# samiwilf/torchrec-oldfork

Hardware: AMD Instinct MI355X
Metric: samples/sec Criteo-1TB DLRM batch 65536 (higher is better)
Workload: dtype f32; 1 GPU; DLRM Criteo-1TB shape: 26 tables (177.9M rows, 84.85 GiB fp32, D=128), 13 dense, pooling factor 1, dense 512-256-128, over 1024-1024-512-256-1, fused exact SGD; global_batch=65536, local_batch=65536, parallelism=mp1: 26 table-wise + 0 row-wise + 0 replicated (data-parallel) tables, dense dp1, ids=uniform, distinct_batches=32, seed=0, data_ranks=1

## Files before the change

include/tbe_hip.h:

```cpp
#ifndef TBE_HIP_H_
#define TBE_HIP_H_

#include <stddef.h>
#include <stdint.h>

#ifdef __cplusplus
extern "C" {
#endif

#define TBE_OK 0
#define TBE_ERR_INVALID_ARGUMENT (-1)
#define TBE_ERR_LAUNCH (-2)
#define TBE_ERR_WORKSPACE (-3)
#define TBE_ERR_UNSUPPORTED (-4)

#define TBE_POOL_SUM 0
#define TBE_POOL_MEAN 1
#define TBE_POOL_NONE 2

#define TBE_OPT_EXACT_SGD 0
#define TBE_OPT_EXACT_ROWWISE_ADAGRAD 1
#define TBE_OPT_ADAM 2
#define TBE_OPT_EXACT_ADAGRAD 3
#define TBE_OPT_DENSE_GRAD 100
// ... 145 lines not shown

int tbe_dlrm_interaction_forward_f32(const float* dense, const float* sparse, int32_t B,
                                     int32_t F, int32_t D, float* out, int64_t out_row_stride,
                                     void* stream);
int tbe_dlrm_interaction_backward_f32(const float* dense, const float* sparse,
                                      const float* grad_out, int64_t grad_row_stride, int32_t B, int32_t F, int32_t D,
                                      float* grad_dense, float* grad_sparse, void* stream);

size_t tbe_relu_backward_bias_grad_workspace_bytes(int64_t B, int32_t N);
int tbe_relu_backward_bias_grad_f32(const float* grad_out, const float* act, int64_t B, int32_t N,
                                    float* grad_in, float* bias_grad, void* workspace,
                                    size_t workspace_bytes, void* stream);

size_t tbe_weighted_colsum_workspace_bytes(int64_t B, int32_t N);
int tbe_weighted_colsum_f32(const float* x, const float* w, int64_t B, int32_t N, float* out,
                            void* workspace, size_t workspace_bytes, void* stream);

int64_t tbe_colsum_row_blocks(int64_t B, int32_t N);
int tbe_relu_backward_bias_partials_f32(const float* grad_out, const float* act, int64_t B, int32_t N,
                                        float* grad_in, float* partial, size_t partial_bytes, void* stream);
int tbe_weighted_colsum_partials_f32(const float* x, const float* w, int64_t B, int32_t N, float* partial,
                                     size_t partial_bytes, void* stream);

int tbe_multi_chunk_sum_f32(const int64_t* seg_table, int32_t nseg, int64_t max_numel, float* dst, float scale,
                            void* stream);
int tbe_multi_chunk_sum_host_table_f32(const int64_t* host_seg_table, int32_t nseg, int64_t max_numel, float* dst,
                                       float scale, void* stream);

size_t tbe_bce_with_logits_workspace_bytes(void);
int tbe_bce_with_logits_f32(const float* logits, const void* labels, int32_t label_elem_size, int64_t B, float* loss,
                            float* dlogits, void* workspace, size_t workspace_bytes, void* stream);

int tbe_jagged_2d_to_dense_f32(const float* values, const int64_t* offsets, int32_t B,
                               int32_t D, int32_t max_L, float* dense, void* stream);

int tbe_dense_to_jagged_2d_f32(const float* dense, const int64_t* offsets, int32_t B, int32_t D,
                               int32_t max_L, int64_t N, float* values, void* stream);

int tbe_offsets_range(const int64_t* offsets, int64_t n, int64_t range_size, int64_t* out,
                      void* stream);

int tbe_copy_rows(const void* src, int64_t src_rows, const int32_t* rows, int32_t n_rows,
                  int64_t row_bytes, void* dst, void* stream);

#ifdef __cplusplus
}
// ... 3 lines not shown
```

torchrec-oldfork_amd/csrc/mlp_epilogue.hip:

```cpp
#include <algorithm>
#include <cstring>

#include "common.hpp"

namespace tbe {

__host__ __device__ inline int rows_per_block(int N) { return N >= 512 ? 256 : 64; }

template <int TX>
__global__ __launch_bounds__(256) void drelu_bgrad_kernel(const float* __restrict__ gy, const float* __restrict__ act,
                                                          float* __restrict__ gx, float* __restrict__ partial,
                                                          int64_t B, int N) {
  constexpr int TY = 256 / TX;
  __shared__ float4 red[TY][TX];
  const int tx = threadIdx.x % TX;
  const int ty = threadIdx.x / TX;
  const int col = (blockIdx.x * TX + tx) * 4;
  const int rpb = rows_per_block(N);
  const int64_t row0 = static_cast<int64_t>(blockIdx.y) * rpb;
  const int64_t row1 = min(B, row0 + rpb);
  float4 acc = make_float4(0.f, 0.f, 0.f, 0.f);
  if (col < N) {
#pragma unroll 4
    for (int64_t r = row0 + ty; r < row1; r += TY) {
// ... 219 lines not shown
    }
  }
  red[threadIdx.x] = acc;
  __syncthreads();
  for (int o = 128; o > 0; o >>= 1) {
    if (static_cast<int>(threadIdx.x) < o) red[threadIdx.x] += red[threadIdx.x + o];
    __syncthreads();
  }
  if (threadIdx.x == 0) {
    __hip_atomic_store(&partial[blockIdx.x], red[0], __ATOMIC_RELAXED, __HIP_MEMORY_SCOPE_AGENT);
    __threadfence();
    is_last = atomicAdd(ticket, 1u) == static_cast<unsigned>(nblk - 1);
  }
  __syncthreads();
  if (is_last && threadIdx.x == 0) {
    __threadfence();
    float tot = 0.f;
    for (int b = 0; b < nblk; ++b) tot += __hip_atomic_load(&partial[b], __ATOMIC_RELAXED, __HIP_MEMORY_SCOPE_AGENT);
    *loss = tot * invB;
    *ticket = 0u;
  }
}

}

using namespace tbe;

extern "C" size_t tbe_relu_backward_bias_grad_workspace_bytes(int64_t B, int32_t N) {
  if (B <= 0 || N <= 0) return 256;
  const int rpb = rows_per_block(N);
  return align_up(static_cast<size_t>((B + rpb - 1) / rpb) * N * sizeof(float), 256);
}

extern "C" int tbe_relu_backward_bias_grad_f32(const float* grad_out, const float* act, int64_t B, int32_t N,
                                               float* grad_in, float* bias_grad, void* workspace,
                                               size_t workspace_bytes, void* stream) {
  TBE_REQUIRE(B >= 0 && N > 0 && (N & 3) == 0, "tbe_relu_backward_bias_grad_f32: N=%d must be a positive multiple of 4", N);
  TBE_REQUIRE(bias_grad != nullptr, "tbe_relu_backward_bias_grad_f32: null bias_grad");
  hipStream_t st = static_cast<hipStream_t>(stream);
  if (B == 0) {
    if (hipMemsetAsync(bias_grad, 0, sizeof(float) * N, st) != hipSuccess) return TBE_ERR_LAUNCH;
    return TBE_OK;
  }
  TBE_REQUIRE(grad_out && act && grad_in && workspace, "tbe_relu_backward_bias_grad_f32: null pointer");
  TBE_REQUIRE(((reinterpret_cast<uintptr_t>(grad_out) | reinterpret_cast<uintptr_t>(act) |
                reinterpret_cast<uintptr_t>(grad_in) | reinterpret_cast<uintptr_t>(workspace)) & 15) == 0,
// ... 88 lines not shown

extern "C" int tbe_weighted_colsum_partials_f32(const float* x, const float* w, int64_t B, int32_t N, float* partial,
                                                size_t partial_bytes, void* stream) {
  TBE_REQUIRE(B > 0 && N > 0 && (N & 3) == 0, "tbe_weighted_colsum_partials_f32: B > 0 and N a positive multiple of 4 required");
  TBE_REQUIRE(x && w && partial, "tbe_weighted_colsum_partials_f32: null pointer");
  TBE_REQUIRE(((reinterpret_cast<uintptr_t>(x) | reinterpret_cast<uintptr_t>(partial)) & 15) == 0,
              "tbe_weighted_colsum_partials_f32: tensors must be 16-B aligned");
  const int64_t nrb = tbe_colsum_row_blocks(B, N);
  TBE_REQUIRE(nrb <= 65535, "tbe_weighted_colsum_partials_f32: B=%lld too large", (long long)B);
  TBE_REQUIRE(partial_bytes >= static_cast<size_t>(nrb) * N * sizeof(float), "tbe_weighted_colsum_partials_f32: partial too small");
  hipStream_t st = static_cast<hipStream_t>(stream);
  const int vecs = N / 4;
  if (vecs >= 64) {
    hipLaunchKernelGGL(wcolsum_kernel<64>, dim3((vecs + 63) / 64, static_cast<unsigned>(nrb)), dim3(256), 0, st, x, w, partial, B, N);
  } else if (vecs >= 32) {
    hipLaunchKernelGGL(wcolsum_kernel<32>, dim3((vecs + 31) / 32, static_cast<unsigned>(nrb)), dim3(256), 0, st, x, w, partial, B, N);
  } else {
    hipLaunchKernelGGL(wcolsum_kernel<16>, dim3((vecs + 15) / 16, static_cast<unsigned>(nrb)), dim3(256), 0, st, x, w, partial, B, N);
  }
  TBE_CHECK_LAUNCH("tbe_weighted_colsum_partials_f32");
  return TBE_OK;
}

extern "C" int tbe_multi_chunk_sum_f32(const int64_t* seg_table, int32_t nseg, int64_t max_numel, float* dst, float scale,
                                       void* stream) {
  TBE_REQUIRE(nseg >= 0 && max_numel >= 0, "tbe_multi_chunk_sum_f32: bad sizes");
  if (nseg == 0 || max_numel == 0) return TBE_OK;
  TBE_REQUIRE(seg_table && dst, "tbe_multi_chunk_sum_f32: null pointer");
  TBE_REQUIRE(nseg <= 65535, "tbe_multi_chunk_sum_f32: more than 65535 segments");
  static_assert(sizeof(ChunkSeg) == 4 * sizeof(int64_t), "segment table layout");
  const int64_t tiles = (max_numel + 255) / 256;
  TBE_REQUIRE(tiles < (1ll << 31), "tbe_multi_chunk_sum_f32: segment too long");
  hipLaunchKernelGGL(multi_chunk_sum_kernel, dim3(static_cast<unsigned>(tiles), static_cast<unsigned>(nseg)), dim3(256), 0,
                     static_cast<hipStream_t>(stream), reinterpret_cast<const ChunkSeg*>(seg_table), dst, scale);
  TBE_CHECK_LAUNCH("tbe_multi_chunk_sum_f32");
  return TBE_OK;
}

extern "C" int tbe_multi_chunk_sum_host_table_f32(const int64_t* host_seg_table, int32_t nseg, int64_t max_numel, float* dst,
                                                  float scale, void* stream) {
  TBE_REQUIRE(nseg >= 0 && nseg <= kChunkSegsByValue && max_numel >= 0,
              "tbe_multi_chunk_sum_host_table_f32: 0 <= nseg <= %d required", kChunkSegsByValue);
  if (nseg == 0 || max_numel == 0) return TBE_OK;
  TBE_REQUIRE(host_seg_table != nullptr, "tbe_multi_chunk_sum_host_table_f32: null table");
  ChunkSegs32 segs{};
  memcpy(segs.s, host_seg_table, static_cast<size_t>(nseg) * sizeof(ChunkSeg));
// ... 31 lines not shown
```

torchrec-oldfork_amd/fbgemm_gpu/_lib.py:

```python
import ctypes
import os
from typing import Optional

import torch

_HERE = os.path.dirname(os.path.abspath(__file__))
LIB_PATH = os.path.normpath(os.path.join(_HERE, "..", "lib", "libtbe_hip.so"))

c_void_p = ctypes.c_void_p
c_i32 = ctypes.c_int32
c_i64 = ctypes.c_int64
c_size = ctypes.c_size_t
c_float = ctypes.c_float


class OptimizerArgs(ctypes.Structure):

    _fields_ = [
        ("optimizer", c_i32),
        ("learning_rate", c_float),
        ("eps", c_float),
        ("weight_decay", c_float),
        ("beta1", c_float),
        ("beta2", c_float),
# ... 88 lines not shown
    "tbe_pooled_exchange_unpack": (
        ctypes.c_int,
        [c_void_p, c_void_p, c_void_p, c_void_p, c_void_p, c_void_p, c_void_p, c_i32, c_i32, c_i32,
         c_i32, c_i32, c_float, c_void_p]),
    "tbe_pooled_exchange_pack": (
        ctypes.c_int,
        [c_void_p, c_void_p, c_void_p, c_void_p, c_void_p, c_void_p, c_void_p, c_i32, c_i32, c_i32,
         c_i32, c_i32, c_float, c_void_p]),
    "tbe_dlrm_interaction_forward_f32": (
        ctypes.c_int, [c_void_p, c_void_p, c_i32, c_i32, c_i32, c_void_p, c_i64, c_void_p]),
    "tbe_dlrm_interaction_backward_f32": (
        ctypes.c_int, [c_void_p, c_void_p, c_void_p, c_i64, c_i32, c_i32, c_i32, c_void_p, c_void_p, c_void_p]),
    "tbe_relu_backward_bias_grad_workspace_bytes": (c_size, [c_i64, c_i32]),
    "tbe_relu_backward_bias_grad_f32": (
        ctypes.c_int, [c_void_p, c_void_p, c_i64, c_i32, c_void_p, c_void_p, c_void_p, c_size, c_void_p]),
    "tbe_weighted_colsum_workspace_bytes": (c_size, [c_i64, c_i32]),
    "tbe_weighted_colsum_f32": (
        ctypes.c_int, [c_void_p, c_void_p, c_i64, c_i32, c_void_p, c_void_p, c_size, c_void_p]),
    "tbe_colsum_row_blocks": (c_i64, [c_i64, c_i32]),
    "tbe_relu_backward_bias_partials_f32": (
        ctypes.c_int, [c_void_p, c_void_p, c_i64, c_i32, c_void_p, c_void_p, c_size, c_void_p]),
    "tbe_weighted_colsum_partials_f32": (
        ctypes.c_int, [c_void_p, c_void_p, c_i64, c_i32, c_void_p, c_size, c_void_p]),
    "tbe_multi_chunk_sum_f32": (ctypes.c_int, [c_void_p, c_i32, c_i64, c_void_p, c_float, c_void_p]),
    "tbe_multi_chunk_sum_host_table_f32": (ctypes.c_int, [c_void_p, c_i32, c_i64, c_void_p, c_float, c_void_p]),
    "tbe_bce_with_logits_workspace_bytes": (c_size, []),
    "tbe_bce_with_logits_f32": (
        ctypes.c_int, [c_void_p, c_void_p, c_i32, c_i64, c_void_p, c_void_p, c_void_p, c_size, c_void_p]),
    "tbe_jagged_2d_to_dense_f32": (
        ctypes.c_int, [c_void_p, c_void_p, c_i32, c_i32, c_i32, c_void_p, c_void_p]),
    "tbe_dense_to_jagged_2d_f32": (
        ctypes.c_int, [c_void_p, c_void_p, c_i32, c_i32, c_i32, c_i64, c_void_p, c_void_p]),
    "tbe_offsets_range": (ctypes.c_int, [c_void_p, c_i64, c_i64, c_void_p, c_void_p]),
    "tbe_copy_rows": (ctypes.c_int, [c_void_p, c_i64, c_void_p, c_i32, c_i64, c_void_p, c_void_p]),
}

_lib: Optional[ctypes.CDLL] = None


def load() -> ctypes.CDLL:
    global _lib
    if _lib is not None:
        return _lib
    if not os.path.exists(LIB_PATH):
        raise ImportError(
            f"{LIB_PATH} is missing: the MI355X HIP extension has not been built. "
# ... 76 lines not shown
```

torchrec-oldfork_amd/torchrec_amd/distributed/_device_ops.py:

```python
import torch

from fbgemm_gpu import _lib
from fbgemm_gpu._lib import check, ptr, require_gpu, stream_ptr

_def = torch.library.Library("tbe_hip", "DEF")
_def.define("pooled_exchange_unpack(Tensor recv, Tensor feat_out_col, Tensor feat_src, Tensor feat_slab_col, "
            "Tensor slab_offset, Tensor slab_stride, int B_local, int D_total, bool vec, float scale) -> Tensor")
_def.define("pooled_exchange_unpack_into(Tensor recv, Tensor feat_out_col, Tensor feat_src, Tensor feat_slab_col, "
            "Tensor slab_offset, Tensor slab_stride, int B_local, int D_total, bool vec, float scale, Tensor(a!) out) -> Tensor(a!)")
_def.define("pooled_exchange_pack(Tensor grad, Tensor feat_out_col, Tensor feat_src, Tensor feat_slab_col, "
            "Tensor slab_offset, Tensor slab_stride, int numel, bool vec, float scale) -> Tensor")
_def.define("pooled_exchange_pack_into(Tensor grad, Tensor feat_out_col, Tensor feat_src, Tensor feat_slab_col, "
            "Tensor slab_offset, Tensor slab_stride, bool vec, float scale, Tensor(a!) send) -> Tensor(a!)")
_def.define("a2a_pooled_unpack(Tensor recv, Tensor dim_sum_per_rank, int B_local, int D_total, bool vec, float scale) -> Tensor")
_def.define("a2a_pooled_pack(Tensor grad, Tensor dim_sum_per_rank, bool vec, float scale) -> Tensor")
_def.define("relu_backward_bias_grad(Tensor grad_out, Tensor act) -> (Tensor, Tensor)")
_def.define("weighted_colsum(Tensor x, Tensor w) -> Tensor")
_def.define("copy_rows(Tensor src, Tensor rows) -> Tensor")
_def.define("relu_backward_bias_partials(Tensor grad_out, Tensor act) -> (Tensor, Tensor)")
_def.define("weighted_colsum_partials(Tensor x, Tensor w) -> Tensor")
_def.define("multi_chunk_sum(Tensor seg_table, int nseg, int max_numel, Tensor(a!) dst, float scale) -> Tensor(a!)")
_def.define("bce_with_logits(Tensor logits, Tensor labels) -> (Tensor, Tensor)")
_impl = torch.library.Library("tbe_hip", "IMPL", "CUDA")


def _copy_rows(src, rows):
    dev = require_gpu(src, rows)
    if src.dim() != 2 or not src.is_contiguous() or rows.dtype != torch.int32 or rows.dim() != 1:
        raise RuntimeError(f"copy_rows: need a contiguous 2-D src and int32 rows, got {tuple(src.shape)} / {rows.dtype}")
    out = src.new_empty((rows.numel(), src.shape[1]))
    lib = _lib.load()
    with torch.cuda.device(dev):
        check(lib.tbe_copy_rows(ptr(src), src.shape[0], ptr(rows), rows.numel(), src.shape[1] * src.element_size(), ptr(out),
                                stream_ptr(dev)), "tbe_copy_rows")
    return out


def _weighted_colsum(x, w):
    from fbgemm_gpu._lib import workspace

    dev = require_gpu(x, w)
    if x.dim() != 2 or w.numel() != x.shape[0] or x.dtype != torch.float32 or w.dtype != torch.float32:
        raise RuntimeError(f"weighted_colsum: need float32 x [B, N] and w [B], got {tuple(x.shape)} and {tuple(w.shape)}")
# ... 35 lines not shown
    grad_out, act = grad_out.contiguous(), act.contiguous()
    B, N = grad_out.shape
    lib = _lib.load()
    gx = torch.empty_like(grad_out)
    partial = torch.empty((lib.tbe_colsum_row_blocks(B, N), N), dtype=torch.float32, device=dev)
    with torch.cuda.device(dev):
        check(lib.tbe_relu_backward_bias_partials_f32(ptr(grad_out), ptr(act), B, N, ptr(gx), ptr(partial),
                                                      partial.numel() * 4, stream_ptr(dev)), "tbe_relu_backward_bias_partials_f32")
    return gx, partial


def _weighted_colsum_partials(x, w):
    dev = require_gpu(x, w)
    if x.dim() != 2 or w.numel() != x.shape[0] or x.dtype != torch.float32 or w.dtype != torch.float32:
        raise RuntimeError(f"weighted_colsum_partials: need float32 x [B, N] and w [B], got {tuple(x.shape)} and {tuple(w.shape)}")
    x, w = x.contiguous(), w.contiguous().view(-1)
    B, N = x.shape
    lib = _lib.load()
    partial = torch.empty((lib.tbe_colsum_row_blocks(B, N), N), dtype=torch.float32, device=dev)
    with torch.cuda.device(dev):
        check(lib.tbe_weighted_colsum_partials_f32(ptr(x), ptr(w), B, N, ptr(partial), partial.numel() * 4, stream_ptr(dev)),
              "tbe_weighted_colsum_partials_f32")
    return partial


def _multi_chunk_sum(seg_table, nseg, max_numel, dst, scale):
    dev = require_gpu(seg_table, dst)
    if seg_table.dtype != torch.int64 or not seg_table.is_contiguous() or seg_table.numel() != 4 * nseg:
        raise RuntimeError("multi_chunk_sum: seg_table must be a contiguous int64 [nseg, 4] device tensor")
    if dst.dtype != torch.float32 or not dst.is_contiguous():
        raise RuntimeError("multi_chunk_sum: dst must be a contiguous float32 tensor")
    with torch.cuda.device(dev):
        check(_lib.load().tbe_multi_chunk_sum_f32(ptr(seg_table), nseg, max_numel, ptr(dst), scale, stream_ptr(dev)),
              "tbe_multi_chunk_sum_f32")
    return dst


_bce_ws = {}


def _bce_with_logits(logits, labels):
    dev = require_gpu(logits, labels)
    if logits.dim() != 1 or labels.shape != logits.shape or logits.dtype != torch.float32:
        raise RuntimeError(f"bce_with_logits: need float32 logits [B] and labels [B], got {tuple(logits.shape)} / {tuple(labels.shape)}")
    if labels.dtype not in (torch.float32, torch.int64):
        labels = labels.float()
# ... 68 lines not shown
    return send


def _pack_into(grad, feat_out_col, feat_src, feat_slab_col, slab_offset, slab_stride, vec, scale, send):
    dev = require_gpu(grad, feat_out_col, feat_src, feat_slab_col, slab_offset, slab_stride, send)
    if grad.dim() != 2 or not grad.is_contiguous() or grad.dtype != torch.float32:
        raise RuntimeError("pooled_exchange_pack_into: grad must be a contiguous float32 [B_local, D_total] matrix")
    if send.dtype != torch.float32 or not send.is_contiguous():
        raise RuntimeError("pooled_exchange_pack_into: send must be a contiguous float32 buffer")
    B_local, D_total = grad.shape
    with torch.cuda.device(dev):
        check(_lib.load().tbe_pooled_exchange_pack(
            ptr(grad), ptr(send), ptr(feat_out_col), ptr(feat_src), ptr(feat_slab_col), ptr(slab_offset),
            ptr(slab_stride), feat_src.numel(), slab_offset.numel(), B_local, D_total, int(vec), scale,
            stream_ptr(dev)), "tbe_pooled_exchange_pack")
    return send


_impl.impl("relu_backward_bias_grad", _relu_backward_bias_grad)
_impl.impl("weighted_colsum", _weighted_colsum)
_impl.impl("copy_rows", _copy_rows)
_impl.impl("relu_backward_bias_partials", _relu_backward_bias_partials)
_impl.impl("weighted_colsum_partials", _weighted_colsum_partials)
_impl.impl("multi_chunk_sum", _multi_chunk_sum)
_impl.impl("bce_with_logits", _bce_with_logits)
_impl.impl("pooled_exchange_unpack", _unpack)
_impl.impl("pooled_exchange_unpack_into", _unpack_into)
_impl.impl("pooled_exchange_pack", _pack)
_impl.impl("pooled_exchange_pack_into", _pack_into)
_impl.impl("a2a_pooled_unpack", _simple_unpack)
_impl.impl("a2a_pooled_pack", _simple_pack)
```

torchrec-oldfork_amd/torchrec_amd/models/dlrm.py:

```python
import os
from typing import Dict, List, Optional, Tuple

import torch
from torch import nn

from ..modules.mlp import MLP, LinearOut
from ..profiling import label
from ..sparse.jagged_tensor import KeyedJaggedTensor, KeyedTensor


class SparseArch(nn.Module):

    def __init__(self, embedding_bag_collection: nn.Module) -> None:
        super().__init__()
        self.embedding_bag_collection = embedding_bag_collection
        cfgs = embedding_bag_collection.embedding_bag_configs
        assert cfgs, "Embedding bag collection cannot be empty!"
        self.D: int = cfgs[0].embedding_dim
        self._sparse_feature_names: List[str] = [n for c in cfgs for n in c.feature_names]
        self.F: int = len(self._sparse_feature_names)

    def start(self, features: KeyedJaggedTensor):
        return self.embedding_bag_collection(features)

# ... 110 lines not shown
        self.register_buffer("triu_indices", torch.triu_indices(self.F + 1, self.F + 1, offset=1), persistent=False)

    def forward(self, dense_features: torch.Tensor, sparse_features: torch.Tensor) -> torch.Tensor:
        if self.F <= 0:
            return dense_features
        if self.fused and _fused_interaction_ok(dense_features, sparse_features):
            return _FusedDotInteraction.apply(dense_features, sparse_features, self.pad_rows, self.grad_sinks)
        combined = torch.cat((dense_features.unsqueeze(1), sparse_features), dim=1)
        interactions = torch.bmm(combined, combined.transpose(1, 2))
        flat = interactions[:, self.triu_indices[0], self.triu_indices[1]]
        return torch.cat((dense_features, flat), dim=1)


class OverArch(nn.Module):
    def __init__(self, in_features: int, layer_sizes: List[int], device: Optional[torch.device] = None) -> None:
        super().__init__()
        if len(layer_sizes) <= 1:
            raise ValueError("OverArch must have multiple layers.")
        self.model = nn.Sequential(
            MLP(in_features, layer_sizes[:-1], bias=True, activation="relu", device=device),
            LinearOut(layer_sizes[-2], layer_sizes[-1], bias=True, device=device))

    def forward(self, features: torch.Tensor) -> torch.Tensor:
        return self.model(features)


class DLRM(nn.Module):
    def __init__(self, embedding_bag_collection: nn.Module, dense_in_features: int,
                 dense_arch_layer_sizes: List[int], over_arch_layer_sizes: List[int],
                 dense_device: Optional[torch.device] = None) -> None:
        super().__init__()
        cfgs = embedding_bag_collection.embedding_bag_configs
        assert len(cfgs) > 0, "At least one embedding bag is required"
        D = cfgs[0].embedding_dim
        assert all(c.embedding_dim == D for c in cfgs), "All EmbeddingBagConfigs must have the same dimension"
        if dense_arch_layer_sizes[-1] != D:
            raise ValueError(f"embedding_bag_collection dimension ({D}) and final dense arch layer size "
                             f"({dense_arch_layer_sizes[-1]}) must match.")
        self.sparse_arch = SparseArch(embedding_bag_collection)
        F = self.sparse_arch.F
        self.dense_arch = DenseArch(dense_in_features, dense_arch_layer_sizes, device=dense_device)
        self.inter_arch = InteractionArch(F)
        over_in = D + (F + 1) * F // 2
        self.over_arch = OverArch(over_in, over_arch_layer_sizes, device=dense_device)
        if dense_device is not None:
            self.inter_arch.to(dense_device)

# ... 489 lines not shown
```

torchrec-oldfork_amd/torchrec_amd/modules/mlp.py:

```python
from typing import Callable, List, Optional, Union

import torch
from torch import nn


class _DeferredWgrad:

    pending: Optional[list] = None
    partials_ok: bool = False

    @classmethod
    def compute(cls, gy: torch.Tensor, x: torch.Tensor, c: int) -> torch.Tensor:
        B = x.shape[0]
        if c > 1 and B % c == 0:
            return torch.bmm(gy.view(c, B // c, -1).transpose(1, 2), x.view(c, B // c, -1)).sum(dim=0)
        return gy.t() @ x

    @classmethod
    def compute_partials(cls, gy: torch.Tensor, x: torch.Tensor, c: int) -> torch.Tensor:
        B = x.shape[0]
        if c > 1 and B % c == 0:
            return torch.bmm(gy.view(c, B // c, -1).transpose(1, 2), x.view(c, B // c, -1))
        return (gy.t() @ x).unsqueeze(0)

    @classmethod
    def stashing(cls, t: torch.Tensor) -> bool:
        return cls.pending is not None and t.is_cuda and torch.cuda.is_current_stream_capturing()


class _LinearSplitKWgrad(torch.autograd.Function):

    @staticmethod
    def forward(ctx, x, weight, bias, chunks, fuse_relu):
        ctx.chunks = chunks
        ctx.has_bias = bias is not None
        ctx.fuse_relu = fuse_relu
        ctx.weight_param = weight if (weight.is_leaf and weight.requires_grad) else None
        ctx.bias_param = bias if (bias is not None and bias.is_leaf and bias.requires_grad) else None
        if fuse_relu:
            out = torch._addmm_activation(bias, x, weight.t(), use_gelu=False)
            ctx.save_for_backward(x, weight, out)
            return out
        ctx.save_for_backward(x, weight)
        return torch.nn.functional.linear(x, weight, bias)

    @staticmethod
    def backward(ctx, gy):
        gb = None
        gb_deferred = False
        if ctx.fuse_relu:
            x, weight, out = ctx.saved_tensors
            if ctx.has_bias and gy.dtype == torch.float32 and out.shape[1] % 4 == 0:
                from ..distributed import _device_ops
                if (_DeferredWgrad.partials_ok and ctx.bias_param is not None and ctx.needs_input_grad[2]
                        and _DeferredWgrad.stashing(gy)):
                    gy, part = torch.ops.tbe_hip.relu_backward_bias_partials(gy, out)
                    _DeferredWgrad.pending.append(("p", ctx.bias_param, part))
                    gb_deferred = True
                else:
                    gy, gb = torch.ops.tbe_hip.relu_backward_bias_grad(gy, out)
            else:
                gy = torch.ops.aten.threshold_backward(gy.contiguous(), out, 0.0)
        else:
            x, weight = ctx.saved_tensors
            gy = gy.contiguous()
        gx = None
        if ctx.needs_input_grad[0]:
            if x.dim() == 2 and x.stride(1) == 1 and x.stride(0) > x.shape[1] and x.stride(0) % 4 == 0:
                gx = gy.new_empty((x.shape[0], x.stride(0)))[:, :x.shape[1]]
                torch.mm(gy, weight, out=gx)
            else:
                gx = gy @ weight
        c = ctx.chunks
        w = ctx.weight_param
        if w is not None and ctx.needs_input_grad[1] and _DeferredWgrad.stashing(gy):
            _DeferredWgrad.pending.append(("w", w, gy, x, c))
            gw = None
        else:
            gw = _DeferredWgrad.compute(gy, x, c)
        if gb is None and ctx.has_bias and not gb_deferred:
            gb = gy.sum(dim=0)
        return gx, gw, gb, None, None


class _LinearOneOutput(torch.autograd.Function):

    @staticmethod
    def forward(ctx, x, weight, bias):
        ctx.save_for_backward(x, weight)
        ctx.has_bias = bias is not None
        ctx.weight_param = weight if (weight.is_leaf and weight.requires_grad) else None
        return torch.nn.functional.linear(x, weight, bias)

    @staticmethod
    def backward(ctx, gy):
        from ..distributed import _device_ops

        x, weight = ctx.saved_tensors
        gy = gy.contiguous()
        gx = gy @ weight if ctx.needs_input_grad[0] else None
        if _DeferredWgrad.partials_ok and ctx.weight_param is not None and _DeferredWgrad.stashing(gy):
            part = torch.ops.tbe_hip.weighted_colsum_partials(x, gy.view(-1))
            _DeferredWgrad.pending.append(("p", ctx.weight_param, part.view(part.shape[0], 1, -1)))
            gw = None
        else:
            gw = torch.ops.tbe_hip.weighted_colsum(x, gy.view(-1)).view(1, -1)
        gb = gy.sum(dim=0) if ctx.has_bias else None
        return gx, gw, gb


class LinearOut(nn.Linear):

    def forward(self, input: torch.Tensor) -> torch.Tensor:
        if (self.out_features == 1 and input.is_cuda and input.dim() == 2 and input.dtype == torch.float32
                and self.in_features % 4 == 0 and torch.is_grad_enabled() and self.weight.requires_grad):
            return _LinearOneOutput.apply(input, self.weight, self.bias)
        return super().forward(input)


def _wgrad_chunks(batch: int, out_f: int, in_f: int) -> int:
    tiles = max(1, (out_f + 127) // 128) * max(1, (in_f + 127) // 128)
    c = 1
    while tiles * c < 256 and c < 32 and batch % (2 * c) == 0 and batch // (2 * c) >= 1024:
        c *= 2
    return c


class Perceptron(nn.Module):
    def __init__(self, in_size: int, out_size: int, bias: bool = True,
                 activation: Union[nn.Module, Callable[[torch.Tensor], torch.Tensor]] = torch.relu,
                 device: Optional[torch.device] = None) -> None:
        super().__init__()
        self._in_size, self._out_size = in_size, out_size
        self._linear = nn.Linear(in_size, out_size, bias=bias, device=device)
        self._activation_fn = activation

    def forward(self, input: torch.Tensor) -> torch.Tensor:
        lin = self._linear
        if input.is_cuda and input.dim() == 2 and torch.is_grad_enabled() and lin.weight.requires_grad:
            c = _wgrad_chunks(input.shape[0], self._out_size, self._in_size)
            relu = self._activation_fn is torch.relu and lin.bias is not None
            if c > 1 or relu:
                y = _LinearSplitKWgrad.apply(input, lin.weight, lin.bias, c, relu)
                return y if relu else self._activation_fn(y)
        return self._activation_fn(lin(input))


class MLP(nn.Module):
    def __init__(self, in_size: int, layer_sizes: List[int], bias: bool = True,
                 activation: Union[str, Callable] = torch.relu, device: Optional[torch.device] = None) -> None:
        super().__init__()
        if activation == "relu":
            activation = torch.relu
        elif activation == "sigmoid":
            activation = torch.sigmoid
        sizes = [in_size] + list(layer_sizes)
        self._mlp = nn.Sequential(*[
            Perceptron(sizes[i], sizes[i + 1], bias=bias, activation=activation, device=device)
            for i in range(len(layer_sizes))])

    def forward(self, input: torch.Tensor) -> torch.Tensor:
        return self._mlp(input)
```

Baseline: 7.711 million samples/s.

## Fuse MLP dgrad GEMM with next layer's ReLU backward and bias-grad partials

Adds a custom MFMA fp32 GEMM kernel that computes the input gradient of a linear layer and, in its epilogue, applies the previous layer's ReLU mask and emits per-row-block column sums as bias-grad partials. The partials are passed backward through a token object so the preceding layer skips its separate relu-backward/bias-reduction pass. A second fused kernel handles the 1-output final layer, computing gx, bias partials and weight partials in one pass. This removes extra full reads and writes of activation gradients, but swaps the vendor GEMM for a hand-written one that may be slower for large shapes.

```diff
diff --git a/include/tbe_hip.h b/include/tbe_hip.h
--- a/include/tbe_hip.h
+++ b/include/tbe_hip.h
@@ -191,6 +191,17 @@
 int tbe_weighted_colsum_partials_f32(const float* x, const float* w, int64_t B, int32_t N, float* partial,
                                      size_t partial_bytes, void* stream);
 
+int tbe_linear_dgrad_drelu_supported(int64_t M, int32_t N, int32_t K);
+int64_t tbe_linear_dgrad_drelu_row_blocks(int64_t M);
+int tbe_linear_dgrad_drelu_f32(const float* grad_out, const float* weight, const float* x, int64_t M, int32_t N,
+                               int32_t K, float* grad_in, float* partial, size_t partial_bytes, void* stream);
+
+int tbe_colsum_partials_f32(const float* partial, int64_t nblocks, int32_t N, float* out, void* stream);
+
+int tbe_one_output_backward_f32(const float* x, const float* grad_out, const float* weight, int64_t B, int32_t N,
+                                float* grad_in, float* bias_partial, float* weight_partial, size_t partial_bytes,
+                                void* stream);
+
 int tbe_multi_chunk_sum_f32(const int64_t* seg_table, int32_t nseg, int64_t max_numel, float* dst, float scale,
                             void* stream);
 int tbe_multi_chunk_sum_host_table_f32(const int64_t* host_seg_table, int32_t nseg, int64_t max_numel, float* dst,
diff --git a/torchrec-oldfork_amd/csrc/mlp_epilogue.hip b/torchrec-oldfork_amd/csrc/mlp_epilogue.hip
--- a/torchrec-oldfork_amd/csrc/mlp_epilogue.hip
+++ b/torchrec-oldfork_amd/csrc/mlp_epilogue.hip
@@ -265,6 +265,196 @@
   }
 }
 
+
+constexpr int kDgBM = 128, kDgBN = 128, kDgBK = 32;
+constexpr int kDgLdA = kDgBK + 4;
+constexpr int kDgLdB = kDgBN + 4;
+constexpr int kDgAFloats = kDgBM * kDgLdA;
+constexpr int kDgBFloats = kDgBK * kDgLdB;
+constexpr int kDgLdsFloats = 2 * (kDgAFloats + kDgBFloats);
+
+using f32x16 = __attribute__((ext_vector_type(16))) float;
+
+__global__ __launch_bounds__(256) void dgrad_drelu_kernel(const float* __restrict__ gm, const float* __restrict__ w,
+                                                          const float* __restrict__ x, float* __restrict__ gx,
+                                                          float* __restrict__ partial, int64_t M, int N, int K) {
+  __shared__ __attribute__((aligned(16))) float lds[kDgLdsFloats];
+  const int nnt = N / kDgBN;
+  const unsigned nwg = gridDim.x;
+  unsigned lid = blockIdx.x;
+  if ((nwg & 7u) == 0) lid = (blockIdx.x & 7u) * (nwg >> 3) + (blockIdx.x >> 3);
+  const int64_t mt = lid / nnt;
+  const int n0 = static_cast<int>(lid % nnt) * kDgBN;
+  const int64_t m0 = mt * kDgBM;
+  const int t = threadIdx.x;
+  const int lane = t & 63;
+  const int wave = t >> 6;
+  const int wm = wave >> 1, wn = wave & 1;
+  const int li = lane & 31, lh = lane >> 5;
+
+  const float* ga[4];
+#pragma unroll
+  for (int j = 0; j < 4; ++j) {
+    const int64_t r = min<int64_t>(m0 + t / 8 + 32 * j, M - 1);
+    ga[j] = gm + r * K + (t % 8) * 4;
+  }
+  const float* gb = w + static_cast<int64_t>(t / 32) * N + n0 + (t % 32) * 4;
+  float4 ra[4], rb[4];
+  auto load_tile = [&](int k0) {
+#pragma unroll
+    for (int j = 0; j < 4; ++j) ra[j] = ld4(ga[j] + k0);
+#pragma unroll
+    for (int j = 0; j < 4; ++j) rb[j] = ld4(gb + static_cast<int64_t>(k0 + 8 * j) * N);
+  };
+  auto store_tile = [&](int buf) {
+    float* As = lds + buf * kDgAFloats;
+    float* Bs = lds + 2 * kDgAFloats + buf * kDgBFloats;
+#pragma unroll
+    for (int j = 0; j < 4; ++j) *reinterpret_cast<float4*>(As + (t / 8 + 32 * j) * kDgLdA + (t % 8) * 4) = ra[j];
+#pragma unroll
+    for (int j = 0; j < 4; ++j) *reinterpret_cast<float4*>(Bs + (t / 32 + 8 * j) * kDgLdB + (t % 32) * 4) = rb[j];
+  };
+
+  f32x16 acc[2][2];
+#pragma unroll
+  for (int a = 0; a < 2; ++a)
+#pragma unroll
+    for (int b = 0; b < 2; ++b)
+#pragma unroll
+      for (int r = 0; r < 16; ++r) acc[a][b][r] = 0.f;
+
+  auto compute_tile = [&](int buf) {
+    const float* As = lds + buf * kDgAFloats;
+    const float* Bs = lds + 2 * kDgAFloats + buf * kDgBFloats;
+#pragma unroll
+    for (int c = 0; c < kDgBK / 16; ++c) {
+      float a[2][8], b[2][8];
+#pragma unroll
+      for (int tm = 0; tm < 2; ++tm) {
+        const float* p = As + (wm * 64 + tm * 32 + li) * kDgLdA + 16 * c + 8 * lh;
+        const float4 lo = *reinterpret_cast<const float4*>(p);
+        const float4 hi = *reinterpret_cast<const float4*>(p + 4);
+        a[tm][0] = lo.x; a[tm][1] = lo.y; a[tm][2] = lo.z; a[tm][3] = lo.w;
+        a[tm][4] = hi.x; a[tm][5] = hi.y; a[tm][6] = hi.z; a[tm][7] = hi.w;
+      }
+#pragma unroll
+      for (int tn = 0; tn < 2; ++tn)
+#pragma unroll
+        for (int s = 0; s < 8; ++s) b[tn][s] = Bs[(16 * c + 8 * lh + s) * kDgLdB + wn * 64 + tn * 32 + li];
+#pragma unroll
+      for (int s = 0; s < 8; ++s)
+#pragma unroll
+        for (int tm = 0; tm < 2; ++tm)
+#pragma unroll
+          for (int tn = 0; tn < 2; ++tn)
+            acc[tm][tn] = __builtin_amdgcn_mfma_f32_32x32x2f32(a[tm][s], b[tn][s], acc[tm][tn], 0, 0, 0);
+    }
+  };
+
+  const int col = n0 + wn * 64 + li;
+  auto out_row = [&](int tm, int r) -> int64_t { return m0 + wm * 64 + tm * 32 + (r & 3) + 8 * (r >> 2) + 4 * lh; };
+
+  const int nk = K / kDgBK;
+  load_tile(0);
+  store_tile(0);
+  __syncthreads();
+  for (int kt = 0; kt + 1 < nk; ++kt) {
+    load_tile((kt + 1) * kDgBK);
+    compute_tile(kt & 1);
+    store_tile((kt + 1) & 1);
+    __syncthreads();
+  }
+  float xm[2][2][16];
+#pragma unroll
+  for (int tm = 0; tm < 2; ++tm)
+#pragma unroll
+    for (int r = 0; r < 16; ++r) {
+      const int64_t row = min<int64_t>(out_row(tm, r), M - 1);
+#pragma unroll
+      for (int tn = 0; tn < 2; ++tn) xm[tm][tn][r] = x[row * N + col + tn * 32];
+    }
+  compute_tile((nk - 1) & 1);
+
+  float cs[2] = {0.f, 0.f};
+#pragma unroll
+  for (int tm = 0; tm < 2; ++tm)
+#pragma unroll
+    for (int r = 0; r < 16; ++r) {
+      const int64_t row = out_row(tm, r);
+      if (row < M) {
+#pragma unroll
+        for (int tn = 0; tn < 2; ++tn) {
+          const float g = xm[tm][tn][r] > 0.f ? acc[tm][tn][r] : 0.f;
+          gx[row * N + col + tn * 32] = g;
+          cs[tn] += g;
+        }
+      }
+    }
+  __syncthreads();
+  float* red = lds;
+#pragma unroll
+  for (int tn = 0; tn < 2; ++tn) {
+    const float o = __shfl_xor(cs[tn], 32);
+    if (lh == 0) red[wm * kDgBN + wn * 64 + tn * 32 + li] = cs[tn] + o;
+  }
+  __syncthreads();
+  if (t < kDgBN) partial[mt * N + n0 + t] = red[t] + red[kDgBN + t];
+}
+
+template <int TX>
+__global__ __launch_bounds__(256) void one_output_backward_kernel(const float* __restrict__ x, const float* __restrict__ dy,
+                                                                  const float* __restrict__ w, float* __restrict__ gx,
+                                                                  float* __restrict__ pbias, float* __restrict__ pw,
+                                                                  int64_t B, int N) {
+  constexpr int TY = 256 / TX;
+  __shared__ float4 red[2][TY][TX];
+  const int tx = threadIdx.x % TX;
+  const int ty = threadIdx.x / TX;
+  const int col = (blockIdx.x * TX + tx) * 4;
+  const int rpb = rows_per_block(N);
+  const int64_t row0 = static_cast<int64_t>(blockIdx.y) * rpb;
+  const int64_t row1 = min(B, row0 + rpb);
+  float4 ab = make_float4(0.f, 0.f, 0.f, 0.f);
+  float4 aw = make_float4(0.f, 0.f, 0.f, 0.f);
+  if (col < N) {
+    const float4 wv = ld4(w + col);
+#pragma unroll 4
+    for (int64_t r = row0 + ty; r < row1; r += TY) {
+      const float4 v = ld4(x + r * N + col);
+      const float s = dy[r];
+      aw.x = fmaf(s, v.x, aw.x);
+      aw.y = fmaf(s, v.y, aw.y);
+      aw.z = fmaf(s, v.z, aw.z);
+      aw.w = fmaf(s, v.w, aw.w);
+      float4 g;
+      g.x = v.x > 0.f ? s * wv.x : 0.f;
+      g.y = v.y > 0.f ? s * wv.y : 0.f;
+      g.z = v.z > 0.f ? s * wv.z : 0.f;
+      g.w = v.w > 0.f ? s * wv.w : 0.f;
+      st4(gx + r * N + col, g);
+      ab.x += g.x;
+      ab.y += g.y;
+      ab.z += g.z;
+      ab.w += g.w;
+    }
+  }
+  red[0][ty][tx] = ab;
+  red[1][ty][tx] = aw;
+  __syncthreads();
+  if (ty < 2 && col < N) {
+    float4 s = red[ty][0][tx];
+#pragma unroll
+    for (int y = 1; y < TY; ++y) {
+      const float4 o = red[ty][y][tx];
+      s.x += o.x;
+      s.y += o.y;
+      s.z += o.z;
+      s.w += o.w;
+    }
+    st4((ty == 0 ? pbias : pw) + static_cast<int64_t>(blockIdx.y) * N + col, s);
+  }
+}
+
 }
 
 using namespace tbe;
@@ -399,6 +589,70 @@
   return TBE_OK;
 }
 
+extern "C" int tbe_linear_dgrad_drelu_supported(int64_t M, int32_t N, int32_t K) {
+  return M > 0 && N > 0 && K > 0 && N % kDgBN == 0 && K % kDgBK == 0 && (M + kDgBM - 1) / kDgBM * (N / kDgBN) < (1ll << 31);
+}
+
+extern "C" int64_t tbe_linear_dgrad_drelu_row_blocks(int64_t M) { return M > 0 ? (M + kDgBM - 1) / kDgBM : 0; }
+
+extern "C" int tbe_linear_dgrad_drelu_f32(const float* grad_out, const float* weight, const float* x, int64_t M, int32_t N,
+                                          int32_t K, float* grad_in, float* partial, size_t partial_bytes, void* stream) {
+  TBE_REQUIRE(tbe_linear_dgrad_drelu_supported(M, N, K),
+              "tbe_linear_dgrad_drelu_f32: M=%lld N=%d K=%d unsupported (M > 0, N %% %d == 0, K %% %d == 0 required)",
+              (long long)M, N, K, kDgBN, kDgBK);
+  TBE_REQUIRE(grad_out && weight && x && grad_in && partial, "tbe_linear_dgrad_drelu_f32: null pointer");
+  TBE_REQUIRE(((reinterpret_cast<uintptr_t>(grad_out) | reinterpret_cast<uintptr_t>(weight) | reinterpret_cast<uintptr_t>(x) |
+                reinterpret_cast<uintptr_t>(grad_in) | reinterpret_cast<uintptr_t>(partial)) & 15) == 0,
+              "tbe_linear_dgrad_drelu_f32: tensors must be 16-B aligned");
+  const int64_t nrb = tbe_linear_dgrad_drelu_row_blocks(M);
+  TBE_REQUIRE(partial_bytes >= static_cast<size_t>(nrb) * N * sizeof(float), "tbe_linear_dgrad_drelu_f32: partial too small");
+  const int64_t nwg = nrb * (N / kDgBN);
+  hipLaunchKernelGGL(dgrad_drelu_kernel, dim3(static_cast<unsigned>(nwg)), dim3(256), 0, static_cast<hipStream_t>(stream),
+                     grad_out, weight, x, grad_in, partial, M, N, K);
+  TBE_CHECK_LAUNCH("tbe_linear_dgrad_drelu_f32");
+  return TBE_OK;
+}
+
+extern "C" int tbe_colsum_partials_f32(const float* partial, int64_t nblocks, int32_t N, float* out, void* stream) {
+  TBE_REQUIRE(nblocks >= 0 && N > 0, "tbe_colsum_partials_f32: nblocks=%lld N=%d", (long long)nblocks, N);
+  TBE_REQUIRE(out != nullptr && (nblocks == 0 || partial != nullptr), "tbe_colsum_partials_f32: null pointer");
+  hipStream_t st = static_cast<hipStream_t>(stream);
+  if (nblocks == 0) {
+    if (hipMemsetAsync(out, 0, sizeof(float) * N, st) != hipSuccess) return TBE_ERR_LAUNCH;
+    return TBE_OK;
+  }
+  hipLaunchKernelGGL(colsum_partials_kernel, dim3((N + 63) / 64), dim3(256), 0, st, partial, nblocks, N, out);
+  TBE_CHECK_LAUNCH("tbe_colsum_partials_f32");
+  return TBE_OK;
+}
+
+extern "C" int tbe_one_output_backward_f32(const float* x, const float* grad_out, const float* weight, int64_t B, int32_t N,
+                                           float* grad_in, float* bias_partial, float* weight_partial, size_t partial_bytes,
+                                           void* stream) {
+  TBE_REQUIRE(B > 0 && N > 0 && (N & 3) == 0, "tbe_one_output_backward_f32: B > 0 and N a positive multiple of 4 required");
+  TBE_REQUIRE(x && grad_out && weight && grad_in && bias_partial && weight_partial, "tbe_one_output_backward_f32: null pointer");
+  TBE_REQUIRE(((reinterpret_cast<uintptr_t>(x) | reinterpret_cast<uintptr_t>(weight) | reinterpret_cast<uintptr_t>(grad_in) |
+                reinterpret_cast<uintptr_t>(bias_partial) | reinterpret_cast<uintptr_t>(weight_partial)) & 15) == 0,
+              "tbe_one_output_backward_f32: tensors must be 16-B aligned");
+  const int64_t nrb = tbe_colsum_row_blocks(B, N);
+  TBE_REQUIRE(nrb <= 65535, "tbe_one_output_backward_f32: B=%lld too large", (long long)B);
+  TBE_REQUIRE(partial_bytes >= static_cast<size_t>(nrb) * N * sizeof(float), "tbe_one_output_backward_f32: partial too small");
+  hipStream_t st = static_cast<hipStream_t>(stream);
+  const int vecs = N / 4;
+  if (vecs >= 64) {
+    hipLaunchKernelGGL(one_output_backward_kernel<64>, dim3((vecs + 63) / 64, static_cast<unsigned>(nrb)), dim3(256), 0, st, x,
+                       grad_out, weight, grad_in, bias_partial, weight_partial, B, N);
+  } else if (vecs >= 32) {
+    hipLaunchKernelGGL(one_output_backward_kernel<32>, dim3((vecs + 31) / 32, static_cast<unsigned>(nrb)), dim3(256), 0, st, x,
+                       grad_out, weight, grad_in, bias_partial, weight_partial, B, N);
+  } else {
+    hipLaunchKernelGGL(one_output_backward_kernel<16>, dim3((vecs + 15) / 16, static_cast<unsigned>(nrb)), dim3(256), 0, st, x,
+                       grad_out, weight, grad_in, bias_partial, weight_partial, B, N);
+  }
+  TBE_CHECK_LAUNCH("tbe_one_output_backward_f32");
+  return TBE_OK;
+}
+
 extern "C" int tbe_multi_chunk_sum_f32(const int64_t* seg_table, int32_t nseg, int64_t max_numel, float* dst, float scale,
                                        void* stream) {
   TBE_REQUIRE(nseg >= 0 && max_numel >= 0, "tbe_multi_chunk_sum_f32: bad sizes");
diff --git a/torchrec-oldfork_amd/fbgemm_gpu/_lib.py b/torchrec-oldfork_amd/fbgemm_gpu/_lib.py
--- a/torchrec-oldfork_amd/fbgemm_gpu/_lib.py
+++ b/torchrec-oldfork_amd/fbgemm_gpu/_lib.py
@@ -134,6 +134,13 @@
         ctypes.c_int, [c_void_p, c_void_p, c_i64, c_i32, c_void_p, c_void_p, c_size, c_void_p]),
     "tbe_weighted_colsum_partials_f32": (
         ctypes.c_int, [c_void_p, c_void_p, c_i64, c_i32, c_void_p, c_size, c_void_p]),
+    "tbe_linear_dgrad_drelu_supported": (ctypes.c_int, [c_i64, c_i32, c_i32]),
+    "tbe_linear_dgrad_drelu_row_blocks": (c_i64, [c_i64]),
+    "tbe_linear_dgrad_drelu_f32": (
+        ctypes.c_int, [c_void_p, c_void_p, c_void_p, c_i64, c_i32, c_i32, c_void_p, c_void_p, c_size, c_void_p]),
+    "tbe_colsum_partials_f32": (ctypes.c_int, [c_void_p, c_i64, c_i32, c_void_p, c_void_p]),
+    "tbe_one_output_backward_f32": (
+        ctypes.c_int, [c_void_p, c_void_p, c_void_p, c_i64, c_i32, c_void_p, c_void_p, c_void_p, c_size, c_void_p]),
     "tbe_multi_chunk_sum_f32": (ctypes.c_int, [c_void_p, c_i32, c_i64, c_void_p, c_float, c_void_p]),
     "tbe_multi_chunk_sum_host_table_f32": (ctypes.c_int, [c_void_p, c_i32, c_i64, c_void_p, c_float, c_void_p]),
     "tbe_bce_with_logits_workspace_bytes": (c_size, []),
diff --git a/torchrec-oldfork_amd/torchrec_amd/distributed/_device_ops.py b/torchrec-oldfork_amd/torchrec_amd/distributed/_device_ops.py
--- a/torchrec-oldfork_amd/torchrec_amd/distributed/_device_ops.py
+++ b/torchrec-oldfork_amd/torchrec_amd/distributed/_device_ops.py
@@ -19,6 +19,9 @@
 _def.define("copy_rows(Tensor src, Tensor rows) -> Tensor")
 _def.define("relu_backward_bias_partials(Tensor grad_out, Tensor act) -> (Tensor, Tensor)")
 _def.define("weighted_colsum_partials(Tensor x, Tensor w) -> Tensor")
+_def.define("linear_dgrad_drelu_partials(Tensor grad_out, Tensor weight, Tensor x) -> (Tensor, Tensor)")
+_def.define("colsum_partials(Tensor partial) -> Tensor")
+_def.define("one_output_backward_partials(Tensor x, Tensor grad_out, Tensor weight) -> (Tensor, Tensor, Tensor)")
 _def.define("multi_chunk_sum(Tensor seg_table, int nseg, int max_numel, Tensor(a!) dst, float scale) -> Tensor(a!)")
 _def.define("bce_with_logits(Tensor logits, Tensor labels) -> (Tensor, Tensor)")
 _impl = torch.library.Library("tbe_hip", "IMPL", "CUDA")
@@ -100,6 +103,59 @@
         check(lib.tbe_weighted_colsum_partials_f32(ptr(x), ptr(w), B, N, ptr(partial), partial.numel() * 4, stream_ptr(dev)),
               "tbe_weighted_colsum_partials_f32")
     return partial
+
+
+def linear_dgrad_drelu_supported(M, N, K):
+    return bool(_lib.load().tbe_linear_dgrad_drelu_supported(M, N, K))
+
+
+def _linear_dgrad_drelu_partials(grad_out, weight, x):
+    dev = require_gpu(grad_out, weight, x)
+    if (grad_out.dim() != 2 or weight.dim() != 2 or x.dim() != 2 or grad_out.shape[1] != weight.shape[0]
+            or x.shape != (grad_out.shape[0], weight.shape[1])
+            or any(t.dtype != torch.float32 for t in (grad_out, weight, x))):
+        raise RuntimeError(f"linear_dgrad_drelu_partials: need float32 grad_out [M, K], weight [K, N], x [M, N], got "
+                           f"{tuple(grad_out.shape)}, {tuple(weight.shape)}, {tuple(x.shape)}")
+    grad_out, weight, x = grad_out.contiguous(), weight.contiguous(), x.contiguous()
+    M, K = grad_out.shape
+    N = weight.shape[1]
+    lib = _lib.load()
+    gx = grad_out.new_empty((M, N))
+    partial = grad_out.new_empty((lib.tbe_linear_dgrad_drelu_row_blocks(M), N))
+    with torch.cuda.device(dev):
+        check(lib.tbe_linear_dgrad_drelu_f32(ptr(grad_out), ptr(weight), ptr(x), M, N, K, ptr(gx), ptr(partial),
+                                             partial.numel() * 4, stream_ptr(dev)), "tbe_linear_dgrad_drelu_f32")
+    return gx, partial
+
+
+def _colsum_partials(partial):
+    dev = require_gpu(partial)
+    if partial.dim() != 2 or partial.dtype != torch.float32:
+        raise RuntimeError(f"colsum_partials: need a float32 [row blocks, N] tensor, got {tuple(partial.shape)}")
+    partial = partial.contiguous()
+    out = partial.new_empty(partial.shape[1])
+    with torch.cuda.device(dev):
+        check(_lib.load().tbe_colsum_partials_f32(ptr(partial), partial.shape[0], partial.shape[1], ptr(out),
+                                                  stream_ptr(dev)), "tbe_colsum_partials_f32")
+    return out
+
+
+def _one_output_backward_partials(x, grad_out, weight):
+    dev = require_gpu(x, grad_out, weight)
+    if (x.dim() != 2 or grad_out.numel() != x.shape[0] or weight.numel() != x.shape[1]
+            or any(t.dtype != torch.float32 for t in (x, grad_out, weight))):
+        raise RuntimeError(f"one_output_backward_partials: need float32 x [B, N], grad_out [B], weight [N], got "
+                           f"{tuple(x.shape)}, {tuple(grad_out.shape)}, {tuple(weight.shape)}")
+    x, grad_out, weight = x.contiguous(), grad_out.contiguous().view(-1), weight.contiguous().view(-1)
+    B, N = x.shape
+    lib = _lib.load()
+    gx = torch.empty_like(x)
+    pb = x.new_empty((lib.tbe_colsum_row_blocks(B, N), N))
+    pw = torch.empty_like(pb)
+    with torch.cuda.device(dev):
+        check(lib.tbe_one_output_backward_f32(ptr(x), ptr(grad_out), ptr(weight), B, N, ptr(gx), ptr(pb), ptr(pw),
+                                              pb.numel() * 4, stream_ptr(dev)), "tbe_one_output_backward_f32")
+    return gx, pb, pw
 
 
 def _multi_chunk_sum(seg_table, nseg, max_numel, dst, scale):
@@ -214,6 +270,9 @@
 _impl.impl("copy_rows", _copy_rows)
 _impl.impl("relu_backward_bias_partials", _relu_backward_bias_partials)
 _impl.impl("weighted_colsum_partials", _weighted_colsum_partials)
+_impl.impl("linear_dgrad_drelu_partials", _linear_dgrad_drelu_partials)
+_impl.impl("colsum_partials", _colsum_partials)
+_impl.impl("one_output_backward_partials", _one_output_backward_partials)
 _impl.impl("multi_chunk_sum", _multi_chunk_sum)
 _impl.impl("bce_with_logits", _bce_with_logits)
 _impl.impl("pooled_exchange_unpack", _unpack)
diff --git a/torchrec-oldfork_amd/torchrec_amd/models/dlrm.py b/torchrec-oldfork_amd/torchrec_amd/models/dlrm.py
--- a/torchrec-oldfork_amd/torchrec_amd/models/dlrm.py
+++ b/torchrec-oldfork_amd/torchrec_amd/models/dlrm.py
@@ -156,7 +156,8 @@
             LinearOut(layer_sizes[-2], layer_sizes[-1], bias=True, device=device))
 
     def forward(self, features: torch.Tensor) -> torch.Tensor:
-        return self.model(features)
+        h, tok = self.model[0].forward_with_token(features)
+        return self.model[1](h, relu_in=tok)
 
 
 class DLRM(nn.Module):
diff --git a/torchrec-oldfork_amd/torchrec_amd/modules/mlp.py b/torchrec-oldfork_amd/torchrec_amd/modules/mlp.py
--- a/torchrec-oldfork_amd/torchrec_amd/modules/mlp.py
+++ b/torchrec-oldfork_amd/torchrec_amd/modules/mlp.py
@@ -28,11 +28,39 @@
         return cls.pending is not None and t.is_cuda and torch.cuda.is_current_stream_capturing()
 
 
+class _ReluGradToken:
+
+    __slots__ = ("partial",)
+
+    def __init__(self) -> None:
+        self.partial: Optional[torch.Tensor] = None
+
+
+def _fused_dgrad_ok(gy: torch.Tensor, weight: torch.Tensor, x: torch.Tensor) -> bool:
+    M, K = gy.shape
+    N = weight.shape[1]
+    if gy.dtype != torch.float32 or weight.dtype != torch.float32 or x.dtype != torch.float32 or not x.is_contiguous():
+        return False
+    if K > 512 or M < 4096:
+        return False
+    from ..distributed._device_ops import linear_dgrad_drelu_supported
+    return linear_dgrad_drelu_supported(M, N, K)
+
+
+def _finish_bias_partials(ctx, part: torch.Tensor):
+    if _DeferredWgrad.partials_ok and ctx.bias_param is not None and ctx.needs_input_grad[2] and _DeferredWgrad.stashing(part):
+        _DeferredWgrad.pending.append(("p", ctx.bias_param, part))
+        return None, True
+    return torch.ops.tbe_hip.colsum_partials(part), False
+
+
 class _LinearSplitKWgrad(torch.autograd.Function):
 
     @staticmethod
-    def forward(ctx, x, weight, bias, chunks, fuse_relu):
+    def forward(ctx, x, weight, bias, chunks, fuse_relu, relu_in=None, relu_out=None):
         ctx.chunks = chunks
+        ctx.relu_in = relu_in
+        ctx.relu_out = relu_out
         ctx.has_bias = bias is not None
         ctx.fuse_relu = fuse_relu
         ctx.weight_param = weight if (weight.is_leaf and weight.requires_grad) else None
@@ -50,7 +78,11 @@
         gb_deferred = False
         if ctx.fuse_relu:
             x, weight, out = ctx.saved_tensors
-            if ctx.has_bias and gy.dtype == torch.float32 and out.shape[1] % 4 == 0:
+            tok = ctx.relu_out
+            if tok is not None and tok.partial is not None:
+                part, tok.partial = tok.partial, None
+                gb, gb_deferred = _finish_bias_partials(ctx, part)
+            elif ctx.has_bias and gy.dtype == torch.float32 and out.shape[1] % 4 == 0:
                 from ..distributed import _device_ops
                 if (_DeferredWgrad.partials_ok and ctx.bias_param is not None and ctx.needs_input_grad[2]
                         and _DeferredWgrad.stashing(gy)):
@@ -65,8 +97,13 @@
             x, weight = ctx.saved_tensors
             gy = gy.contiguous()
         gx = None
+        tok = ctx.relu_in
+        if tok is not None:
+            tok.partial = None
         if ctx.needs_input_grad[0]:
-            if x.dim() == 2 and x.stride(1) == 1 and x.stride(0) > x.shape[1] and x.stride(0) % 4 == 0:
+            if tok is not None and _fused_dgrad_ok(gy, weight, x):
+                gx, tok.partial = torch.ops.tbe_hip.linear_dgrad_drelu_partials(gy, weight, x)
+            elif x.dim() == 2 and x.stride(1) == 1 and x.stride(0) > x.shape[1] and x.stride(0) % 4 == 0:
                 gx = gy.new_empty((x.shape[0], x.stride(0)))[:, :x.shape[1]]
                 torch.mm(gy, weight, out=gx)
             else:
@@ -80,13 +117,14 @@
             gw = _DeferredWgrad.compute(gy, x, c)
         if gb is None and ctx.has_bias and not gb_deferred:
             gb = gy.sum(dim=0)
-        return gx, gw, gb, None, None
+        return gx, gw, gb, None, None, None, None
 
 
 class _LinearOneOutput(torch.autograd.Function):
 
     @staticmethod
-    def forward(ctx, x, weight, bias):
+    def forward(ctx, x, weight, bias, relu_in=None):
+        ctx.relu_in = relu_in
         ctx.save_for_backward(x, weight)
         ctx.has_bias = bias is not None
         ctx.weight_param = weight if (weight.is_leaf and weight.requires_grad) else None
@@ -98,23 +136,34 @@
 
         x, weight = ctx.saved_tensors
         gy = gy.contiguous()
-        gx = gy @ weight if ctx.needs_input_grad[0] else None
-        if _DeferredWgrad.partials_ok and ctx.weight_param is not None and _DeferredWgrad.stashing(gy):
-            part = torch.ops.tbe_hip.weighted_colsum_partials(x, gy.view(-1))
-            _DeferredWgrad.pending.append(("p", ctx.weight_param, part.view(part.shape[0], 1, -1)))
-            gw = None
+        tok = ctx.relu_in
+        if tok is not None:
+            tok.partial = None
+        if tok is not None and ctx.needs_input_grad[0] and gy.dtype == torch.float32 and x.is_contiguous():
+            gx, tok.partial, part = torch.ops.tbe_hip.one_output_backward_partials(x, gy.view(-1), weight)
+            if _DeferredWgrad.partials_ok and ctx.weight_param is not None and _DeferredWgrad.stashing(gy):
+                _DeferredWgrad.pending.append(("p", ctx.weight_param, part.view(part.shape[0], 1, -1)))
+                gw = None
+            else:
+                gw = torch.ops.tbe_hip.colsum_partials(part).view(1, -1)
         else:
-            gw = torch.ops.tbe_hip.weighted_colsum(x, gy.view(-1)).view(1, -1)
+            gx = gy @ weight if ctx.needs_input_grad[0] else None
+            if _DeferredWgrad.partials_ok and ctx.weight_param is not None and _DeferredWgrad.stashing(gy):
+                part = torch.ops.tbe_hip.weighted_colsum_partials(x, gy.view(-1))
+                _DeferredWgrad.pending.append(("p", ctx.weight_param, part.view(part.shape[0], 1, -1)))
+                gw = None
+            else:
+                gw = torch.ops.tbe_hip.weighted_colsum(x, gy.view(-1)).view(1, -1)
         gb = gy.sum(dim=0) if ctx.has_bias else None
-        return gx, gw, gb
+        return gx, gw, gb, None
 
 
 class LinearOut(nn.Linear):
 
-    def forward(self, input: torch.Tensor) -> torch.Tensor:
+    def forward(self, input: torch.Tensor, relu_in: Optional[_ReluGradToken] = None) -> torch.Tensor:
         if (self.out_features == 1 and input.is_cuda and input.dim() == 2 and input.dtype == torch.float32
                 and self.in_features % 4 == 0 and torch.is_grad_enabled() and self.weight.requires_grad):
-            return _LinearOneOutput.apply(input, self.weight, self.bias)
+            return _LinearOneOutput.apply(input, self.weight, self.bias, relu_in)
         return super().forward(input)
 
 
@@ -136,14 +185,18 @@
         self._activation_fn = activation
 
     def forward(self, input: torch.Tensor) -> torch.Tensor:
+        return self.forward_with_token(input)[0]
+
+    def forward_with_token(self, input: torch.Tensor, relu_in: Optional[_ReluGradToken] = None):
         lin = self._linear
         if input.is_cuda and input.dim() == 2 and torch.is_grad_enabled() and lin.weight.requires_grad:
             c = _wgrad_chunks(input.shape[0], self._out_size, self._in_size)
             relu = self._activation_fn is torch.relu and lin.bias is not None
-            if c > 1 or relu:
-                y = _LinearSplitKWgrad.apply(input, lin.weight, lin.bias, c, relu)
-                return y if relu else self._activation_fn(y)
-        return self._activation_fn(lin(input))
+            if c > 1 or relu or relu_in is not None:
+                tok = _ReluGradToken() if relu else None
+                y = _LinearSplitKWgrad.apply(input, lin.weight, lin.bias, c, relu, relu_in, tok)
+                return (y, tok) if relu else (self._activation_fn(y), None)
+        return self._activation_fn(lin(input)), None
 
 
 class MLP(nn.Module):
@@ -160,4 +213,10 @@
             for i in range(len(layer_sizes))])
 
     def forward(self, input: torch.Tensor) -> torch.Tensor:
-        return self._mlp(input)
+        return self.forward_with_token(input)[0]
+
+    def forward_with_token(self, input: torch.Tensor):
+        tok = None
+        for p in self._mlp:
+            input, tok = p.forward_with_token(input, tok)
+        return input, tok
```

Measured after the change: 7.799 million samples/s, median of 6. +1.1%, better.
